# TorchIO-project/torchio

Hardware: NVIDIA H100
Metric: augmented voxels/sec on 256^3 fp32 Compose pipeline (higher is better)
Workload: dtype f32

## Files before the change

### torchio_b200/csrc/build.py

```python

from __future__ import annotations

import os
import subprocess
import sys
from concurrent.futures import ThreadPoolExecutor
from pathlib import Path

HERE = Path(__file__).resolve().parent
ROOT = HERE.parent.parent
SOURCES = ["error.cu", "resample.cu", "resample_tile.cu", "resample_fast.cu", "intensity.cu", "fused_intensity.cu",
           "mt19937_jump.cpp", "mt19937.cu", "patches.cu", "stats.cu", "labels.cu"]
HEADERS = [HERE / "common.cuh", HERE / "intensity_common.cuh", HERE / "resample_common.cuh", HERE / "resample_tile.cuh", HERE / "tma.cuh",
           ROOT / "include" / "tio_b200.h",
           Path(__file__).resolve()]
OBJ = HERE / "_obj"
OUT = HERE / "libtio_b200.so"

ARCH = ["-gencode", "arch=compute_90a,code=sm_90a"]
NVCC_FLAGS = [
    *ARCH,
    "-O3", "-std=c++17", "-lineinfo",
    "-Xcompiler", "-fPIC",
    "-Xptxas", "-v",
]


def needs_build() -> bool:
    if not OUT.exists():
        return True
    newest = max(p.stat().st_mtime for p in [*(HERE / s for s in SOURCES), *HEADERS])
    return OUT.stat().st_mtime < newest


def _compile(source: str) -> tuple[str, int, str]:
    src = HERE / source
    obj = OBJ / (Path(source).stem + ".o")
    newest = max(p.stat().st_mtime for p in [src, *HEADERS])
    if obj.exists() and obj.stat().st_mtime >= newest:
        return source, 0, ""
    proc = subprocess.run(["nvcc", *NVCC_FLAGS, "-c", str(src), "-o", str(obj)],
                          capture_output=True, text=True)
    return source, proc.returncode, proc.stdout + proc.stderr


def build(force: bool = False, verbose: bool = False) -> Path:
    if not force and not needs_build():
        return OUT
    OBJ.mkdir(exist_ok=True)
    if force:
        for stale in OBJ.glob("*.o"):
            stale.unlink()
    with ThreadPoolExecutor(max_workers=min(len(SOURCES), os.cpu_count() or 1)) as pool:
        results = list(pool.map(_compile, SOURCES))
    log = "".join(f"==== {name}\n{text}" for name, _, text in results)
    failed = [name for name, code, _ in results if code != 0]
    if verbose or failed:
        sys.stderr.write(log)
    if failed:
        raise RuntimeError(f"nvcc failed for {failed}")
    objects = [str(OBJ / (Path(s).stem + ".o")) for s in SOURCES]
    proc = subprocess.run(["nvcc", *ARCH, "-shared", "-o", str(OUT),
                           *objects], capture_output=True, text=True)
    if proc.returncode != 0:
        sys.stderr.write(proc.stdout + proc.stderr)
        raise RuntimeError(f"nvcc link failed with exit code {proc.returncode}")
    previous = (HERE / "ptxas.log").read_text() if (HERE / "ptxas.log").exists() and not force else ""
    (HERE / "ptxas.log").write_text(log if all(t for _, _, t in results) else previous + log)
    return OUT


if __name__ == "__main__":
    path = build(force="--force" in sys.argv, verbose="--verbose" in sys.argv)
    print(path)
```

### torchio_b200/csrc/mt19937.cu

```cuda
#include "common.cuh"

namespace tio {

constexpr int MT_N = 624, MT_M = 397, MT_DEG = 19937;
constexpr int MT_SEQ = MT_DEG + MT_N;
constexpr int MT_OFFS = (MT_SEQ + 7) / 4 * 4;

__device__ __forceinline__ uint32_t mt_twist(uint32_t a, uint32_t b, uint32_t c) {
  const uint32_t y = (a & 0x80000000u) | (b & 0x7fffffffu);
  return c ^ (y >> 1) ^ ((y & 1u) ? 0x9908b0dfu : 0u);
}

__device__ __forceinline__ uint32_t mt_temper(uint32_t y) {
  y ^= y >> 11;
  y ^= (y << 7) & 0x9d2c5680u;
  y ^= (y << 15) & 0xefc60000u;
  y ^= y >> 18;
  return y;
}

__global__ void mt_seed_kernel(uint32_t seed, uint32_t* __restrict__ states) {
  if (threadIdx.x == 0) {
    uint32_t v = seed;
    states[0] = v;
    for (int j = 1; j < MT_N; ++j) {
      v = 1812433253u * (v ^ (v >> 30)) + (uint32_t)j;
      states[j] = v;
    }
  }
}

struct MtJob { int src, dst, slot; };

__global__ void __launch_bounds__(640)
mt_jump_kernel(uint32_t* __restrict__ states, const uint16_t* __restrict__ polys, int stride,
               int first, int S2, int fine) {
  extern __shared__ __align__(16) uint32_t seq[];
  uint32_t* offs = seq + MT_OFFS;
  MtJob job;
  if (fine) {
    const int q = first + (int)blockIdx.x, r = q % S2;
    if (r == 0) return;
    job = MtJob{q - r, q, r - 1};
  } else {
    const int m = first + (int)blockIdx.x;
    job = MtJob{0, m * S2, (S2 - 1) + (m - 1)};
  }
  const int tid = threadIdx.x;
  const uint32_t* src = states + (size_t)job.src * MT_N;
  for (int t = tid; t < MT_N; t += blockDim.x) seq[t] = src[t];
  __syncthreads();
  for (int base = 0; base + MT_N < MT_SEQ; base += MT_N - MT_M) {
    const int k = base + tid;
    if (tid < MT_N - MT_M && k + MT_N < MT_SEQ)
      seq[k + MT_N] = mt_twist(seq[k], seq[k + 1], seq[k + MT_M]);
    __syncthreads();
  }
  const uint16_t* p = polys + (size_t)job.slot * stride;
  const uint32_t count = p[0] | ((uint32_t)p[1] << 16);
  const char* mine = reinterpret_cast<const char*>(seq + (tid < MT_N ? tid : 0));
  uint32_t acc = 0;
  for (uint32_t c0 = 0; c0 < count; c0 += 2048) {
    const uint32_t chunk = min(2048u, count - c0);
    for (uint32_t t = tid; t < chunk; t += blockDim.x) offs[t] = (uint32_t)p[2 + c0 + t] << 2;
    __syncthreads();
    if (tid < MT_N) {
      const uint4* o4 = reinterpret_cast<const uint4*>(offs);
      const uint32_t quads = chunk >> 2;
#pragma unroll 4
      for (uint32_t t = 0; t < quads; ++t) {
        const uint4 o = o4[t];
        acc ^= *reinterpret_cast<const uint32_t*>(mine + o.x) ^ *reinterpret_cast<const uint32_t*>(mine + o.y);
        acc ^= *reinterpret_cast<const uint32_t*>(mine + o.z) ^ *reinterpret_cast<const uint32_t*>(mine + o.w);
      }
      for (uint32_t t = quads << 2; t < chunk; ++t) acc ^= *reinterpret_cast<const uint32_t*>(mine + offs[t]);
    }
    __syncthreads();
  }
  if (tid < MT_N) states[(size_t)job.dst * MT_N + tid] = acc;
}

__device__ __forceinline__ void sincos_0_2pi(float theta, float& sn, float& cs) {
  const float t = __fmaf_rn(theta, 0.6366197723675814f, 12582912.0f);
  const int j = __float_as_int(t);
  const float jf = __fsub_rn(t, 12582912.0f);
  float r = __fmaf_rn(jf, -1.5707962512969971f, theta);
  r = __fmaf_rn(jf, -7.549789415861596e-08f, r);
  const float r2 = __fmul_rn(r, r);
  float ps = __fmaf_rn(r2, -1.9515295891e-4f, 8.3321608736e-3f);
  ps = __fmaf_rn(ps, r2, -1.6666654611e-1f);
  const float s = __fmaf_rn(__fmul_rn(ps, r2), r, r);
  float pc = __fmaf_rn(r2, 2.443315711809948e-5f, -1.388731625493765e-3f);
  pc = __fmaf_rn(pc, r2, 4.166664568298827e-2f);
  const float c = __fmaf_rn(__fmul_rn(pc, r2), r2, __fmaf_rn(r2, -0.5f, 1.0f));
  const bool swap = j & 1;
  const float a = swap ? c : s, b = swap ? s : c;
  sn = (j & 2) ? -a : a;
  cs = ((j + 1) & 2) ? -b : b;
}

__global__ void __launch_bounds__(320)
mt_normal_kernel(const uint32_t* __restrict__ states, int q_first, unsigned long long L,
                 unsigned long long offset, unsigned long long n, float* __restrict__ z) {
  __shared__ uint32_t s[2 * MT_N];
  const int tid = threadIdx.x;
  const int q = q_first + blockIdx.x;
  const unsigned long long seg_begin = (unsigned long long)q * L;
  const unsigned long long lo = max(seg_begin, offset);
  const unsigned long long hi = min(seg_begin + L, offset + n);
  if (lo >= hi) return;
  const uint32_t* w = states + (size_t)q * MT_N;
  for (int t = tid; t < MT_N; t += blockDim.x) s[t] = w[t];
  __syncthreads();
  constexpr int W = MT_N - MT_M;
  const int blk = tid >> 3, j = tid & 7;
  const int pair = 16 * blk + j;
  const int lo_rel = (int)(lo - seg_begin), hi_rel = (int)(hi - seg_begin);
  const long long seg_to_z = (long long)seg_begin - (long long)offset;
  int flip = 0;
  for (int base = 0; base < hi_rel; base += MT_N, flip ^= 1) {
    const uint32_t* cur = s + flip * MT_N;
    uint32_t* nxt = s + (flip ^ 1) * MT_N;
    if (tid < W) nxt[tid] = mt_twist(cur[tid], cur[tid + 1], cur[tid + MT_M]);
    __syncthreads();
    if (tid < W) nxt[W + tid] = mt_twist(cur[W + tid], cur[W + tid + 1], nxt[tid]);
    __syncthreads();
    if (tid < MT_N - 2 * W) {
      const int k = 2 * W + tid;
      const uint32_t b = (k + 1 < MT_N) ? cur[k + 1] : nxt[0];
      nxt[k] = mt_twist(cur[k], b, nxt[k - W]);
    }
    __syncthreads();
    if (tid < 312 && base + MT_N > lo_rel) {
      const int t0 = base + pair;
      const bool whole = (base >= lo_rel) && (base + MT_N <= hi_rel);
      if (whole || (t0 >= lo_rel && t0 < hi_rel)) {
        const float u1 = (float)(mt_temper(nxt[pair]) & 0xffffffu) * (1.0f / 16777216.0f);
        const float u2 = (float)(mt_temper(nxt[pair + 8]) & 0xffffffu) * (1.0f / 16777216.0f);
        float radius;
        asm("sqrt.approx.ftz.f32 %0, %1;" : "=f"(radius) : "f"(-2.0f * logf(1.0f - u1)));
        const float theta = (float)(6.283185307179586 * (double)u2);
        float sn, cs;
        sincos_0_2pi(theta, sn, cs);
        float* zp = z + (seg_to_z + t0);
        zp[0] = radius * cs;
        zp[8] = radius * sn;
      }
    }
  }
}

}

using namespace tio;

extern "C" size_t tio_randn_mt19937_workspace_bytes(uint64_t offset, uint64_t n) {
  const uint64_t L = 1ull << 20;
  const uint64_t q_hi = (offset + n + L - 1) / L;
  return (size_t)(q_hi + 64) * MT_N * 4;
}

extern "C" int tio_randn_mt19937(uint64_t seed, uint64_t offset, uint64_t n, float* z,
                                 const void* table, void* workspace, size_t workspace_bytes,
                                 void* stream) {
  TIO_CHECK_ARG(z && table && workspace, "tio_randn_mt19937: null pointer");
  TIO_CHECK_ARG(n >= 16 && (n % 16) == 0 && (offset % 16) == 0,
                "tio_randn_mt19937: n and offset must be multiples of 16 (n >= 16)");
  const uint64_t L = 1ull << 20;
  const int S2 = 32, S1 = 64, stride = 10496;
  const uint64_t q_lo = offset / L, q_hi = (offset + n + L - 1) / L;
  TIO_CHECK_ARG(q_hi <= (uint64_t)S1 * S2, "tio_randn_mt19937: stream position beyond %d segments", S1 * S2);
  TIO_CHECK_ARG(workspace_bytes >= tio_randn_mt19937_workspace_bytes(offset, n),
                "tio_randn_mt19937: workspace too small");
  cudaStream_t st = (cudaStream_t)stream;
  uint32_t* states = (uint32_t*)workspace;
  const uint16_t* polys = (const uint16_t*)((const char*)table + 32);
  mt_seed_kernel<<<1, 32, 0, st>>>((uint32_t)seed, states);
  const size_t jump_smem = (size_t)(MT_OFFS + 2048) * 4;
  cudaFuncSetAttribute(mt_jump_kernel, cudaFuncAttributeMaxDynamicSharedMemorySize, (int)jump_smem);
  const int m_lo = (int)(q_lo / S2), m_hi = (int)((q_hi - 1) / S2);
  const int m_first = m_lo > 1 ? m_lo : 1;
  if (m_hi >= m_first)
    mt_jump_kernel<<<m_hi - m_first + 1, 640, jump_smem, st>>>(states, polys, stride, m_first, S2, 0);
  mt_jump_kernel<<<(unsigned)(q_hi - q_lo), 640, jump_smem, st>>>(states, polys, stride, (int)q_lo, S2, 1);
  mt_normal_kernel<<<(unsigned)(q_hi - q_lo), 320, 0, st>>>(states, (int)q_lo, L, offset, n, z);
  TIO_CHECK_LAUNCH();
  return 0;
}
```

### torchio_b200/csrc/mt19937_jump.cpp

```cpp
#include <stdint.h>
#include <string.h>

#include <vector>

#include "../../include/tio_b200.h"

namespace {

constexpr int kDeg = 19937;
constexpr int kWords = (2 * kDeg + 63) / 64 + 1;

struct Bits {
  std::vector<uint64_t> w;
  explicit Bits(int words = kWords) : w(words, 0) {}
  bool get(int i) const { return (w[i >> 6] >> (i & 63)) & 1u; }
  void flip(int i) { w[i >> 6] ^= (uint64_t)1 << (i & 63); }
  void set(int i) { w[i >> 6] |= (uint64_t)1 << (i & 63); }
};

static void xor_shifted(Bits& a, const Bits& b, int s, int nw) {
  const int ws = s >> 6, bs = s & 63;
  const int limit = (int)a.w.size();
  if (bs == 0) {
    for (int i = 0; i < nw && i + ws < limit; ++i) a.w[i + ws] ^= b.w[i];
  } else {
    for (int i = 0; i < nw; ++i) {
      const uint64_t v = b.w[i];
      if (!v) continue;
      if (i + ws < limit) a.w[i + ws] ^= v << bs;
      if (i + ws + 1 < limit) a.w[i + ws + 1] ^= v >> (64 - bs);
    }
  }
}

struct Mt {
  uint32_t s[624];
  int idx;
  void seed(uint32_t v) {
    s[0] = v;
    for (int j = 1; j < 624; ++j) s[j] = 1812433253u * (s[j - 1] ^ (s[j - 1] >> 30)) + (uint32_t)j;
    idx = 624;
  }
  uint32_t raw() {
    if (idx >= 624) {
      for (int k = 0; k < 624; ++k) {
        uint32_t y = (s[k] & 0x80000000u) | (s[(k + 1) % 624] & 0x7fffffffu);
        s[k] = s[(k + 397) % 624] ^ (y >> 1) ^ ((y & 1u) ? 0x9908b0dfu : 0u);
      }
      idx = 0;
    }
    return s[idx++];
  }
};

struct Field {
  Bits phi;
  std::vector<int> phi_terms;

  void reduce(Bits& a) const {
    for (int d = 2 * kDeg; d >= kDeg; --d) {
      if (!a.get(d)) continue;
      const int s = d - kDeg;
      a.flip(d);
      for (int e : phi_terms) a.flip(e + s);
    }
  }
  Bits mul(const Bits& a, const Bits& b) const {
    Bits r;
    const int nw = (kDeg + 63) / 64;
    for (int i = 0; i < kDeg; ++i)
      if (a.get(i)) xor_shifted(r, b, i, nw);
    reduce(r);
    return r;
  }
};

static bool build_field(Field& f) {
  Mt g;
  g.seed(19650218u);
  std::vector<uint8_t> seq(2 * kDeg + 64);
  for (auto& v : seq) v = (uint8_t)(g.raw() & 1u);
  const int n = (int)seq.size();
  const int W = (kDeg + 64) / 64 + 1;
  std::vector<uint64_t> c(W, 0), b(W, 0), t(W, 0), rev(W, 0);
  c[0] = 1;
  b[0] = 1;
  int L = 0, m = 1;
  for (int i = 0; i < n; ++i) {
    for (int k = W - 1; k > 0; --k) rev[k] = (rev[k] << 1) | (rev[k - 1] >> 63);
    rev[0] = (rev[0] << 1) | seq[i];
    uint64_t acc = 0;
    for (int k = 0; k < W; ++k) acc ^= c[k] & rev[k];
    const int d = __builtin_popcountll(acc) & 1;
    if (d) {
      t = c;
      const int ws = m >> 6, bs = m & 63;
      for (int k = 0; k + ws < W; ++k) {
        c[k + ws] ^= b[k] << bs;
        if (bs && k + ws + 1 < W) c[k + ws + 1] ^= b[k] >> (64 - bs);
      }
      if (2 * L <= i) {
        L = i + 1 - L;
        b = t;
        m = 1;
      } else {
        ++m;
      }
    } else {
      ++m;
    }
  }
  if (L != kDeg) return false;
  f.phi = Bits();
  f.phi_terms.clear();
  for (int j = 0; j <= kDeg; ++j)
    if ((c[j >> 6] >> (j & 63)) & 1u) {
      f.phi.set(kDeg - j);
      if (kDeg - j < kDeg) f.phi_terms.push_back(kDeg - j);
    }
  return f.phi.get(kDeg);
}

}

static constexpr uint32_t kMagic = 0x4d544a31u;
static constexpr int kLog2L = 20, kS2 = 32, kS1 = 64;
static constexpr int kStride = 10496;

extern "C" size_t tio_mt19937_table_bytes(void) {
  return 32 + (size_t)((kS2 - 1) + (kS1 - 1)) * kStride * sizeof(uint16_t);
}

extern "C" int tio_mt19937_build_table(void* blob, size_t bytes) {
  if (!blob || bytes < tio_mt19937_table_bytes()) return 1;
  Field f;
  if (!build_field(f)) return 2;
  uint32_t* header = (uint32_t*)blob;
  header[0] = kMagic; header[1] = kLog2L; header[2] = kS2; header[3] = kS1;
  header[4] = (kS2 - 1) + (kS1 - 1); header[5] = kStride; header[6] = header[7] = 0;
  uint16_t* out = (uint16_t*)((char*)blob + 32);
  auto emit = [&](const Bits& p, int slot) -> bool {
    uint16_t* dst = out + (size_t)slot * kStride;
    uint32_t count = 0;
    for (int i = 0; i < kDeg; ++i)
      if (p.get(i)) {
        if (2 + count >= (uint32_t)kStride) return false;
        dst[2 + count++] = (uint16_t)i;
      }
    dst[0] = (uint16_t)(count & 0xffffu);
    dst[1] = (uint16_t)(count >> 16);
    return true;
  };
  Bits h1;
  h1.set(1);
  for (int i = 0; i < kLog2L; ++i) h1 = f.mul(h1, h1);
  Bits cur = h1;
  for (int r = 1; r < kS2; ++r) {
    if (!emit(cur, r - 1)) return 3;
    cur = f.mul(cur, h1);
  }
  const Bits b1 = cur;
  cur = b1;
  for (int m = 1; m < kS1; ++m) {
    if (!emit(cur, (kS2 - 1) + (m - 1))) return 3;
    if (m + 1 < kS1) cur = f.mul(cur, b1);
  }
  return 0;
}

extern "C" int tio_mt19937_apply_poly_host(const void* blob, int slot, const uint32_t* in,
                                           uint32_t* out) {
  const uint32_t* header = (const uint32_t*)blob;
  if (header[0] != kMagic || slot < 0 || slot >= (int)header[4]) return 1;
  const uint16_t* p = (const uint16_t*)((const char*)blob + 32) + (size_t)slot * header[5];
  const uint32_t count = p[0] | ((uint32_t)p[1] << 16);
  std::vector<uint32_t> seq(kDeg + 624 + 8);
  memcpy(seq.data(), in, 624 * 4);
  for (int k = 0; k + 624 < (int)seq.size(); ++k) {
    uint32_t y = (seq[k] & 0x80000000u) | (seq[k + 1] & 0x7fffffffu);
    seq[k + 624] = seq[k + 397] ^ (y >> 1) ^ ((y & 1u) ? 0x9908b0dfu : 0u);
  }
  for (int j = 0; j < 624; ++j) out[j] = 0;
  for (uint32_t t = 0; t < count; ++t) {
    const uint32_t* s = seq.data() + p[2 + t];
    for (int j = 0; j < 624; ++j) out[j] ^= s[j];
  }
  return 0;
}
```

### torchio_b200/ops.py

```python

from __future__ import annotations

import os
import threading

import numpy as np
import torch
from torch import Tensor

from . import _native

DTYPE_CODES = {
    torch.float32: 0, torch.uint8: 1, torch.int8: 2,
    torch.int16: 3, torch.int32: 4, torch.int64: 5,
}
NEAREST, LINEAR, LABEL_PV = 0, 1, 2
FLAG_PASSTHROUGH, FLAG_ELASTIC = 1, 2

_counter = threading.local()


def launches() -> int:
    return getattr(_counter, "n", 0)


def _count(n: int) -> None:
    _counter.n = getattr(_counter, "n", 0) + n


def _stream(t: Tensor) -> int:
    return torch.cuda.current_stream(t.device).cuda_stream


def _ptr(t: Tensor | None):
    return None if t is None else t.data_ptr()


def _require_cuda(t: Tensor, name: str) -> None:
    if not t.is_cuda:
        raise RuntimeError(
            f"torchio_b200.ops.{name}: expected a CUDA tensor (got {t.device});"
            " the kernels have no CPU fallback"
        )
    if t.requires_grad:
        raise NotImplementedError(
            f"torchio_b200.ops.{name}: kernels are forward-only; detach() the input"
        )


class _StagingRing:

    SLOTS = 64
    SLOT_BYTES = 1 << 20

    def __init__(self) -> None:
        self.buffers = [torch.empty(self.SLOT_BYTES, dtype=torch.uint8, pin_memory=True)
                        for _ in range(self.SLOTS)]
        self.events: list = [None] * self.SLOTS
        self.index = 0
        self.lock = threading.Lock()

    def take(self):
        with self.lock:
            i = self.index
            self.index = (i + 1) % self.SLOTS
            pending, self.events[i] = self.events[i], None
        if pending is not None:
            pending.synchronize()
        return i, self.buffers[i]

    def release(self, i: int, device: torch.device) -> None:
        ev = torch.cuda.Event()
        ev.record(torch.cuda.current_stream(device))
        with self.lock:
            self.events[i] = ev


_ring: _StagingRing | None = None
_init_lock = threading.Lock()


def upload(device: torch.device, *arrays):
    global _ring
    specs, offset = [], 0
    for a in arrays:
        if a is None:
            specs.append(None)
            continue
        t = torch.as_tensor(a)
        t = t.contiguous()
        nbytes = t.numel() * t.element_size()
        specs.append((t, offset, nbytes))
        offset += (nbytes + 15) // 16 * 16
    if offset == 0:
        return [None] * len(arrays)
    slot = None
    if torch.cuda.is_available() and offset <= _StagingRing.SLOT_BYTES:
        if _ring is None:
            with _init_lock:
                if _ring is None:
                    _ring = _StagingRing()
        slot, stage = _ring.take()
        stage = stage[:offset]
    else:
        stage = torch.empty(offset, dtype=torch.uint8, pin_memory=torch.cuda.is_available())
    stage_np = stage.numpy()
    for s in specs:
        if s is None:
            continue
        t, off, nbytes = s
        stage_np[off:off + nbytes] = t.reshape(-1).numpy().view(np.uint8)
    if slot is not None:
        dev = torch.empty(offset, dtype=torch.uint8, device=device)
        _native.call("tio_upload", stage.data_ptr(), dev.data_ptr(), offset,
                     torch.cuda.current_stream(dev.device).cuda_stream)
        _count(1)
        _ring.release(slot, torch.device(device))
    else:
        dev = stage.to(device, non_blocking=True)
    out = []
    for s in specs:
        if s is None:
            out.append(None)
            continue
        t, off, nbytes = s
        out.append(dev[off:off + nbytes].view(t.dtype).reshape(t.shape))
    return out


EXACT_COORDS = 0x100
_exact_default = os.environ.get("TIO_B200_EXACT_COORDS", "0") not in ("", "0")


def set_exact_coords(enabled: bool) -> bool:
    global _exact_default
    previous, _exact_default = _exact_default, bool(enabled)
    return previous


def exact_coords_default() -> bool:
    return _exact_default


def resample(
    src: Tensor, mat: Tensor, cp: Tensor | None, flags: Tensor | None,
    spacing_in, spacing_out, *, affine_first: bool, mode: int,
    fill: Tensor | None, out_shape=None, box_hint: int = 0, exact_coords: bool | None = None,
) -> Tensor:
    _require_cuda(src, "resample")
    if src.dtype not in DTYPE_CODES:
        raise TypeError(f"resample: unsupported dtype {src.dtype}")
    src = src.contiguous()
    b, c, i, j, k = src.shape
    oi, oj, ok = (i, j, k) if out_shape is None else out_shape
    dst = torch.empty((b, c, oi, oj, ok), dtype=src.dtype, device=src.device)
    ni = nj = nk = 0
    if cp is not None:
        ni, nj, nk = cp.shape[1:4]
    sp_in = np.asarray(spacing_in, dtype=np.float32)
    sp_out = np.asarray(spacing_out, dtype=np.float32)
    workspace, ws_bytes = None, 0
    tiled = (src.dtype == torch.float32 and mode == LINEAR) or (
        mode in (NEAREST, LABEL_PV) and src.dtype in (torch.uint8, torch.int16, torch.int32))
    if box_hint >= 0 and tiled:
        ws_bytes = _native.lib().tio_resample_workspace_bytes(b, oi, oj, ok)
        workspace = torch.empty(ws_bytes, dtype=torch.uint8, device=src.device)
    with torch.cuda.device(src.device):
        _native.call(
            "tio_resample", _ptr(src), _ptr(dst), DTYPE_CODES[src.dtype],
            b, c, i, j, k, oi, oj, ok, _ptr(mat), _ptr(cp), _ptr(flags), ni, nj, nk,
            sp_in.ctypes.data, sp_out.ctypes.data, int(bool(affine_first)),
            int(mode) | (EXACT_COORDS if (_exact_default if exact_coords is None else exact_coords) else 0),
            _ptr(fill), int(box_hint), _ptr(workspace), ws_bytes, _stream(src),
        )
    _count(2 if workspace is not None else 1)
    return dst


def _label_table(labels: Tensor, dtype: torch.dtype) -> Tensor:
    return labels.to(torch.float32 if dtype == torch.float32 else torch.int64).contiguous()


def onehot(src: Tensor, labels: Tensor) -> Tensor:
    _require_cuda(src, "onehot")
    if src.dtype not in DTYPE_CODES:
        raise TypeError(f"onehot: unsupported dtype {src.dtype}")
    src = src.contiguous()
    b, n = src.shape[0], int(labels.numel())
    vox = src[0].numel()
    table = _label_table(labels, src.dtype)
    dst = torch.empty((b, n, *src.shape[2:]), dtype=torch.float32, device=src.device)
    with torch.cuda.device(src.device):
        _native.call("tio_onehot", _ptr(src), DTYPE_CODES[src.dtype], b, vox, _ptr(table), n, _ptr(dst),
                     _stream(src))
    _count(1)
    return dst


def label_argmax(sampled: Tensor, labels: Tensor, pad_label: float, dtype: torch.dtype) -> Tensor:
    _require_cuda(sampled, "label_argmax")
    if dtype not in DTYPE_CODES:
        raise TypeError(f"label_argmax: unsupported dtype {dtype}")
    sampled = sampled.contiguous()
    b, n = sampled.shape[:2]
    vox = sampled[0, 0].numel()
    table = _label_table(labels, dtype)
    dst = torch.empty((b, 1, *sampled.shape[2:]), dtype=dtype, device=sampled.device)
    with torch.cuda.device(sampled.device):
        _native.call("tio_label_argmax", _ptr(sampled), b, n, vox, _ptr(table), float(pad_label), _ptr(dst),
                     DTYPE_CODES[dtype], _stream(sampled))
    _count(1)
    return dst


def min_sample0(src: Tensor) -> Tensor:
    _require_cuda(src, "min_sample0")
    src = src.contiguous()
    c = src.shape[1]
    n = src[0, 0].numel()
    fill = torch.empty(c, dtype=torch.float32, device=src.device)
    with torch.cuda.device(src.device):
        _native.call("tio_min_sample0", _ptr(src), c, n, _ptr(fill), _stream(src))
    _count(2)
    return fill


def crop_patches(volume: Tensor, corners, size, out: Tensor | None = None) -> Tensor:
    _require_cuda(volume, "crop_patches")
    if volume.ndim != 4:
        raise ValueError(f"crop_patches expects a (C, I, J, K) volume, got {tuple(volume.shape)}")
    volume = volume.contiguous()
    corners = np.ascontiguousarray(np.asarray(corners, dtype=np.int32).reshape(-1, 3))
    n = corners.shape[0]
    c, i, j, k = (int(v) for v in volume.shape)
    pi, pj, pk = (int(v) for v in size)
    if n == 0:
        return volume.new_empty((0, c, pi, pj, pk))
    if corners.min() < 0 or np.any(corners + np.asarray([pi, pj, pk]) > np.asarray([i, j, k])):
        raise ValueError("crop_patches: a patch extends beyond the volume")
    (corners_d,) = upload(volume.device, corners)
    if out is None:
        dst = torch.empty((n, c, pi, pj, pk), dtype=volume.dtype, device=volume.device)
    else:
        dst = out
        if (tuple(dst.shape) != (n, c, pi, pj, pk) or dst.dtype != volume.dtype or dst.device != volume.device
                or not dst.is_contiguous()):
            raise ValueError("crop_patches: `out` must be a contiguous (n, C, *size) block of the volume's dtype/device")
    with torch.cuda.device(volume.device):
        _native.call(
            "tio_crop_patches", _ptr(volume), _ptr(dst), volume.element_size(), c, i, j, k, n,
            _ptr(corners_d), pi, pj, pk, _stream(volume),
        )
    _count(1)
    return dst


PAD_MODES = {"constant": 0, "replicate": 1, "reflect": 2, "circular": 3}


def remap(src: Tensor, out_shape, offsets, *, mode: str = "constant", fill=0, flip: Tensor | None = None,
          out: Tensor | None = None) -> Tensor:
    _require_cuda(src, "remap")
    if src.ndim != 5:
        raise ValueError(f"remap expects (B, C, I, J, K), got {tuple(src.shape)}")
    src = src.contiguous()
    b, c, i, j, k = (int(v) for v in src.shape)
    oi, oj, ok = (int(v) for v in out_shape)
    if out is None:
        dst = torch.empty((b, c, oi, oj, ok), dtype=src.dtype, device=src.device)
    else:
        dst = out
        if (tuple(dst.shape) != (b, c, oi, oj, ok) or dst.dtype != src.dtype or dst.device != src.device
                or not dst.is_contiguous()):
            raise ValueError("remap: `out` must be a contiguous (B, C, *out_shape) block of the source's dtype/device")
    fill_host = torch.tensor([fill]).to(src.dtype)
    with torch.cuda.device(src.device):
        _native.call(
            "tio_remap", _ptr(src), _ptr(dst), src.element_size(), b, c, i, j, k, oi, oj, ok,
            int(offsets[0]), int(offsets[1]), int(offsets[2]), PAD_MODES[mode],
            fill_host.data_ptr(), _ptr(flip), _stream(src),
        )
    _count(1)
    return dst


def bias_field(src: Tensor, coarse: Tensor, identity: Tensor | None, *, divide=False,
               out: Tensor | None = None) -> Tensor:
    _require_cuda(src, "bias_field")
    src = src.contiguous()
    b, c, i, j, k = src.shape
    dst = torch.empty_like(src) if out is None else out
    si, sj, sk = coarse.shape[2:]
    with torch.cuda.device(src.device):
        _native.call(
            "tio_bias_field", _ptr(src), _ptr(dst), b, c, i, j, k, _ptr(coarse), si, sj, sk,
            _ptr(identity), int(bool(divide)), _stream(src),
        )
    _count(1)
    return dst


def blur(src: Tensor, taps: Tensor, radius: Tensor, big_r: int, axes_mask: int,
         identity: Tensor | None) -> Tensor:
    _require_cuda(src, "blur")
    src = src.contiguous()
    b, c, i, j, k = src.shape
    dst = torch.empty_like(src)
    scratch = torch.empty_like(src) if (axes_mask & 6) else None
    with torch.cuda.device(src.device):
        _native.call(
            "tio_blur", _ptr(src), _ptr(dst), _ptr(scratch), b, c, i, j, k, _ptr(taps),
            _ptr(radius), int(big_r), int(axes_mask), _ptr(identity), _stream(src),
        )
    _count(_fused_launches(axes_mask, False))
    return dst


def _fused_launches(axes_mask: int, has_bias: bool) -> int:
    jk = bool(axes_mask & 6)
    march = (not jk) or bool(axes_mask & 1) or has_bias
    return int(jk) + int(march)


def noise(src: Tensor, mean: Tensor, std: Tensor, keep: Tensor | None, z: Tensor,
          z2: Tensor | None = None) -> Tensor:
    _require_cuda(src, "noise")
    src = src.contiguous()
    dst = torch.empty_like(src)
    with torch.cuda.device(src.device):
        _native.call(
            "tio_noise", _ptr(src), _ptr(dst), src.shape[0], src[0].numel(), _ptr(mean),
            _ptr(std), _ptr(keep), _ptr(z), _ptr(z2), _stream(src),
        )
    _count(1)
    return dst


def noise_philox(src: Tensor, mean: Tensor, std: Tensor, keep: Tensor | None, seed: int,
                 rician: bool = False) -> Tensor:
    _require_cuda(src, "noise_philox")
    src = src.contiguous()
    dst = torch.empty_like(src)
    with torch.cuda.device(src.device):
        _native.call(
            "tio_noise_philox", _ptr(src), _ptr(dst), src.shape[0], src[0].numel(),
            _ptr(mean), _ptr(std), _ptr(keep), int(seed), int(bool(rician)), _stream(src),
        )
    _count(1)
    return dst


def gamma(src: Tensor, gam: Tensor) -> Tensor:
    _require_cuda(src, "gamma")
    src = src.contiguous()
    dst = torch.empty_like(src)
    with torch.cuda.device(src.device):
        _native.call(
            "tio_gamma", _ptr(src), _ptr(dst), src.shape[0], src[0].numel(), _ptr(gam),
            _stream(src),
        )
    _count(1)
    return dst


def moments(values: Tensor, mask: Tensor | None = None) -> tuple[float, float, float]:
    _require_cuda(values, "moments")
    values = values.contiguous()
    m8 = None if mask is None else mask.expand_as(values).contiguous().to(torch.uint8)
    out = torch.empty(3, dtype=torch.float64, device=values.device)
    with torch.cuda.device(values.device):
        _native.call("tio_moments", _ptr(values), _ptr(m8), values.numel(), _ptr(out), _stream(values))
    _count(1)
    s, ss, n = out.tolist()
    return s, ss, n


def quantile_neighbours(values: Tensor, qs, mask: Tensor | None = None):
    _require_cuda(values, "quantile_neighbours")
    values = values.contiguous()
    m8 = None if mask is None else mask.expand_as(values).contiguous().to(torch.uint8)
    qs = np.ascontiguousarray(np.asarray(qs, dtype=np.float64).reshape(-1))
    m = int(qs.shape[0])
    dev = values.device
    vals = torch.empty(2 * m, dtype=torch.float32, device=dev)
    out = torch.empty(m + 1, dtype=torch.float64, device=dev)
    ws_bytes = _native.lib().tio_quantiles_workspace_bytes()
    ws = torch.empty(ws_bytes, dtype=torch.uint8, device=dev)
    with torch.cuda.device(dev):
        _native.call("tio_quantiles", _ptr(values), _ptr(m8), values.numel(), qs.ctypes.data, m, _ptr(vals),
                     _ptr(out), out[m:].data_ptr(), _ptr(ws), ws_bytes, _stream(values))
    _count(8)
    host = out.tolist()
    return vals.tolist(), host[:m], int(host[m])


def rescale(src: Tensor, *, lo: float | None = None, hi: float | None = None, sub=None, div=None, mul=None,
            add=None, keep=None) -> Tensor:
    _require_cuda(src, "rescale")
    src = src.contiguous()
    b = src.shape[0]
    flags = (1 if lo is not None else 0)
    tabs = []
    for bit, table in ((2, sub), (4, div), (8, mul), (16, add)):
        if table is None:
            tabs.append(None)
            continue
        flags |= bit
        arr = np.asarray(table, dtype=np.float32).reshape(-1)
        tabs.append(np.ascontiguousarray(np.broadcast_to(arr, (b,)) if arr.size == 1 else arr))
    keep_np = None if keep is None else np.ascontiguousarray(np.asarray(keep, dtype=np.uint8))
    sub_d, div_d, mul_d, add_d, keep_d = upload(src.device, *tabs, keep_np)
    dst = torch.empty_like(src)
    with torch.cuda.device(src.device):
        _native.call("tio_rescale", _ptr(src), _ptr(dst), b, src[0].numel(),
                     float(lo if lo is not None else 0.0), float(hi if hi is not None else 0.0),
                     _ptr(sub_d), _ptr(div_d), _ptr(mul_d), _ptr(add_d), _ptr(keep_d), flags, _stream(src))
    _count(2)
    return dst


def intensity_fused(
    src: Tensor, *, coarse: Tensor | None = None, bias_identity: Tensor | None = None,
    bias_divide: bool = False, taps: Tensor | None = None, radius: Tensor | None = None,
    big_r: int = 0, axes_mask: int = 0, mean: Tensor | None = None, std: Tensor | None = None,
    keep: Tensor | None = None, z: Tensor | None = None, z2: Tensor | None = None,
    philox_seed: int = 0, noise_mode: int = 0, rician: bool = False,
    gamma: Tensor | None = None,
) -> Tensor:
    _require_cuda(src, "intensity_fused")
    src = src.contiguous()
    b, c, i, j, k = src.shape
    dst = torch.empty_like(src)
    jk = taps is not None and (axes_mask & 6)
    scratch = torch.empty_like(src) if jk else None
    si = sj = sk = 0
    if coarse is not None:
        si, sj, sk = coarse.shape[2:]
    with torch.cuda.device(src.device):
        _native.call(
            "tio_intensity_fused", _ptr(src), _ptr(dst), _ptr(scratch), b, c, i, j, k,
            _ptr(coarse), si, sj, sk, _ptr(bias_identity), int(bool(bias_divide)),
            _ptr(taps), _ptr(radius), int(big_r), int(axes_mask),
            _ptr(mean), _ptr(std), _ptr(keep), _ptr(z), _ptr(z2),
            int(philox_seed) & (2**64 - 1), int(noise_mode), int(bool(rician)),
            _ptr(gamma), _stream(src),
        )
    _count(_fused_launches(axes_mask if taps is not None else 0, coarse is not None))
    return dst



_MT_TABLE_FILE = _native.LIB_PATH.parent / "mt19937_jump.bin"
_mt_host_table: Tensor | None = None
_mt_device_tables: dict = {}
_mt_lock = threading.Lock()
MT_MAX_WORDS = 1 << 31


def mt19937_host_table() -> Tensor:
    global _mt_host_table
    with _mt_lock:
        if _mt_host_table is None:
            lib = _native.lib()
            nbytes = lib.tio_mt19937_table_bytes()
            blob = None
            if _MT_TABLE_FILE.exists() and _MT_TABLE_FILE.stat().st_size == nbytes:
                blob = torch.from_numpy(np.fromfile(_MT_TABLE_FILE, dtype=np.uint8))
            if blob is None:
                blob = torch.zeros(nbytes, dtype=torch.uint8)
                _native.call("tio_mt19937_build_table", blob.data_ptr(), nbytes)
                try:
                    blob.numpy().tofile(_MT_TABLE_FILE)
                except OSError:
                    pass
            _mt_host_table = blob
        return _mt_host_table


def _mt_table(device: torch.device) -> Tensor:
    key = (device.type, device.index)
    table = _mt_device_tables.get(key)
    if table is None:
        with _init_lock:
            table = _mt_device_tables.get(key)
            if table is None:
                table = mt19937_host_table().to(device)
                torch.cuda.synchronize(device)
                _mt_device_tables[key] = table
    return table


def randn_mt19937(seed: int, offset: int, n: int, device, out: Tensor | None = None) -> Tensor:
    device = torch.device(device)
    if n < 16 or n % 16 or offset % 16 or offset + n > MT_MAX_WORDS:
        raise ValueError("randn_mt19937: offset and n must be multiples of 16, n >= 16,"
                         " offset + n <= 2**31")
    z = torch.empty(n, dtype=torch.float32, device=device) if out is None else out
    lib = _native.lib()
    ws_bytes = lib.tio_randn_mt19937_workspace_bytes(offset, n)
    workspace = torch.empty(ws_bytes, dtype=torch.uint8, device=device)
    table = _mt_table(device)
    with torch.cuda.device(device):
        _native.call("tio_randn_mt19937", int(seed) & 0xFFFFFFFF, offset, n, _ptr(z), _ptr(table),
                     _ptr(workspace), ws_bytes, torch.cuda.current_stream(device).cuda_stream)
    _count(4)
    return z
```

Measured before the change: 46.64 billion.

## Warp-specialize MT19937 normal generation and split coarse jump across blocks

Restructures the MT19937 normal kernel into producer warps that twist state into a shared-memory ring and consumer warps that temper and apply vectorized Box-Muller. Named barriers let the twist and the transform overlap. The coarse jump polynomial application is split across several blocks per job, with results combined by atomicXor into memset-zeroed states. Segment length doubles (2^21 with 16 fine steps), which halves fine jumps and gives fewer, longer segments. This trades extra shared memory and synchronization complexity against more parallelism, and needs a regenerated jump table whose header is validated in Python.

Result: faster. 50.02 billion (median of 6 runs) (+7.2%).

```diff
diff --git a/torchio_b200/csrc/build.py b/torchio_b200/csrc/build.py
--- a/torchio_b200/csrc/build.py
+++ b/torchio_b200/csrc/build.py
@@ -12,6 +12,7 @@
 SOURCES = ["error.cu", "resample.cu", "resample_tile.cu", "resample_fast.cu", "intensity.cu", "fused_intensity.cu",
            "mt19937_jump.cpp", "mt19937.cu", "patches.cu", "stats.cu", "labels.cu"]
 HEADERS = [HERE / "common.cuh", HERE / "intensity_common.cuh", HERE / "resample_common.cuh", HERE / "resample_tile.cuh", HERE / "tma.cuh",
+           HERE / "mt19937_layout.h",
            ROOT / "include" / "tio_b200.h",
            Path(__file__).resolve()]
 OBJ = HERE / "_obj"
diff --git a/torchio_b200/csrc/mt19937.cu b/torchio_b200/csrc/mt19937.cu
--- a/torchio_b200/csrc/mt19937.cu
+++ b/torchio_b200/csrc/mt19937.cu
@@ -1,4 +1,5 @@
 #include "common.cuh"
+#include "mt19937_layout.h"
 
 namespace tio {
 
@@ -34,16 +35,17 @@
 
 __global__ void __launch_bounds__(640)
 mt_jump_kernel(uint32_t* __restrict__ states, const uint16_t* __restrict__ polys, int stride,
-               int first, int S2, int fine) {
+               int first, int S2, int fine, int parts) {
   extern __shared__ __align__(16) uint32_t seq[];
   uint32_t* offs = seq + MT_OFFS;
+  const int job_idx = (int)blockIdx.x / parts, part = (int)blockIdx.x % parts;
   MtJob job;
   if (fine) {
-    const int q = first + (int)blockIdx.x, r = q % S2;
+    const int q = first + job_idx, r = q % S2;
     if (r == 0) return;
     job = MtJob{q - r, q, r - 1};
   } else {
-    const int m = first + (int)blockIdx.x;
+    const int m = first + job_idx;
     job = MtJob{0, m * S2, (S2 - 1) + (m - 1)};
   }
   const int tid = threadIdx.x;
@@ -58,10 +60,12 @@
   }
   const uint16_t* p = polys + (size_t)job.slot * stride;
   const uint32_t count = p[0] | ((uint32_t)p[1] << 16);
+  const uint32_t t_begin = (uint32_t)((uint64_t)count * part / parts);
+  const uint32_t t_end = (uint32_t)((uint64_t)count * (part + 1) / parts);
   const char* mine = reinterpret_cast<const char*>(seq + (tid < MT_N ? tid : 0));
   uint32_t acc = 0;
-  for (uint32_t c0 = 0; c0 < count; c0 += 2048) {
-    const uint32_t chunk = min(2048u, count - c0);
+  for (uint32_t c0 = t_begin; c0 < t_end; c0 += 2048) {
+    const uint32_t chunk = min(2048u, t_end - c0);
     for (uint32_t t = tid; t < chunk; t += blockDim.x) offs[t] = (uint32_t)p[2 + c0 + t] << 2;
     __syncthreads();
     if (tid < MT_N) {
@@ -77,7 +81,11 @@
     }
     __syncthreads();
   }
-  if (tid < MT_N) states[(size_t)job.dst * MT_N + tid] = acc;
+  if (tid < MT_N) {
+    uint32_t* dst = states + (size_t)job.dst * MT_N + tid;
+    if (parts == 1) *dst = acc;
+    else atomicXor(dst, acc);
+  }
 }
 
 __device__ __forceinline__ void sincos_0_2pi(float theta, float& sn, float& cs) {
@@ -99,52 +107,108 @@
   cs = ((j + 1) & 2) ? -b : b;
 }
 
-__global__ void __launch_bounds__(320)
+__device__ __forceinline__ void mt_box_muller(uint32_t a, uint32_t b, float& zc, float& zs) {
+  const float u1 = (float)(mt_temper(a) & 0xffffffu) * (1.0f / 16777216.0f);
+  const float u2 = (float)(mt_temper(b) & 0xffffffu) * (1.0f / 16777216.0f);
+  float radius;
+  asm("sqrt.approx.ftz.f32 %0, %1;" : "=f"(radius) : "f"(-2.0f * logf(1.0f - u1)));
+  const float theta = (float)(6.283185307179586 * (double)u2);
+  float sn, cs;
+  sincos_0_2pi(theta, sn, cs);
+  zc = radius * cs;
+  zs = radius * sn;
+}
+
+template <int ID, int COUNT>
+__device__ __forceinline__ void mt_bar_sync() {
+  asm volatile("bar.sync %0, %1;" ::"n"(ID), "n"(COUNT) : "memory");
+}
+template <int ID, int COUNT>
+__device__ __forceinline__ void mt_bar_arrive() {
+  asm volatile("bar.arrive %0, %1;" ::"n"(ID), "n"(COUNT) : "memory");
+}
+
+constexpr int MT_ROUND = 4;
+constexpr int MT_RING = 2 * MT_ROUND;
+constexpr int MT_ITEMS = MT_ROUND * MT_N / 8;
+constexpr int MT_PRODUCERS = 256;
+constexpr int MT_CONSUMERS = (MT_ITEMS + 31) / 32 * 32;
+constexpr int MT_THREADS = MT_PRODUCERS + MT_CONSUMERS;
+constexpr int MT_BAR_PROD = 1, MT_BAR_FULL = 2, MT_BAR_EMPTY = 4;
+
+__global__ void __launch_bounds__(MT_THREADS, 2)
 mt_normal_kernel(const uint32_t* __restrict__ states, int q_first, unsigned long long L,
                  unsigned long long offset, unsigned long long n, float* __restrict__ z) {
-  __shared__ uint32_t s[2 * MT_N];
+  __shared__ __align__(16) uint32_t ring[MT_RING * MT_N];
   const int tid = threadIdx.x;
   const int q = q_first + blockIdx.x;
   const unsigned long long seg_begin = (unsigned long long)q * L;
   const unsigned long long lo = max(seg_begin, offset);
   const unsigned long long hi = min(seg_begin + L, offset + n);
   if (lo >= hi) return;
-  const uint32_t* w = states + (size_t)q * MT_N;
-  for (int t = tid; t < MT_N; t += blockDim.x) s[t] = w[t];
-  __syncthreads();
-  constexpr int W = MT_N - MT_M;
-  const int blk = tid >> 3, j = tid & 7;
-  const int pair = 16 * blk + j;
   const int lo_rel = (int)(lo - seg_begin), hi_rel = (int)(hi - seg_begin);
-  const long long seg_to_z = (long long)seg_begin - (long long)offset;
-  int flip = 0;
-  for (int base = 0; base < hi_rel; base += MT_N, flip ^= 1) {
-    const uint32_t* cur = s + flip * MT_N;
-    uint32_t* nxt = s + (flip ^ 1) * MT_N;
-    if (tid < W) nxt[tid] = mt_twist(cur[tid], cur[tid + 1], cur[tid + MT_M]);
-    __syncthreads();
-    if (tid < W) nxt[W + tid] = mt_twist(cur[W + tid], cur[W + tid + 1], nxt[tid]);
-    __syncthreads();
-    if (tid < MT_N - 2 * W) {
-      const int k = 2 * W + tid;
-      const uint32_t b = (k + 1 < MT_N) ? cur[k + 1] : nxt[0];
-      nxt[k] = mt_twist(cur[k], b, nxt[k - W]);
-    }
-    __syncthreads();
-    if (tid < 312 && base + MT_N > lo_rel) {
-      const int t0 = base + pair;
-      const bool whole = (base >= lo_rel) && (base + MT_N <= hi_rel);
-      if (whole || (t0 >= lo_rel && t0 < hi_rel)) {
-        const float u1 = (float)(mt_temper(nxt[pair]) & 0xffffffu) * (1.0f / 16777216.0f);
-        const float u2 = (float)(mt_temper(nxt[pair + 8]) & 0xffffffu) * (1.0f / 16777216.0f);
-        float radius;
-        asm("sqrt.approx.ftz.f32 %0, %1;" : "=f"(radius) : "f"(-2.0f * logf(1.0f - u1)));
-        const float theta = (float)(6.283185307179586 * (double)u2);
-        float sn, cs;
-        sincos_0_2pi(theta, sn, cs);
-        float* zp = z + (seg_to_z + t0);
-        zp[0] = radius * cs;
-        zp[8] = radius * sn;
+  const int rounds = ((hi_rel + MT_N - 1) / MT_N + MT_ROUND - 1) / MT_ROUND;
+  if (tid < MT_PRODUCERS) {
+    constexpr int W = MT_N - MT_M;
+    const uint32_t* w = states + (size_t)q * MT_N;
+    uint32_t* start = ring + (MT_RING - 1) * MT_N;
+    for (int t = tid; t < MT_N; t += MT_PRODUCERS) start[t] = w[t];
+    mt_bar_sync<MT_BAR_PROD, MT_PRODUCERS>();
+    for (int r = 0; r < rounds; ++r) {
+      if (r >= 2) {
+        if (r & 1) mt_bar_sync<MT_BAR_EMPTY + 1, MT_THREADS>();
+        else mt_bar_sync<MT_BAR_EMPTY, MT_THREADS>();
+      }
+      for (int i = 0; i < MT_ROUND; ++i) {
+        const int b = r * MT_ROUND + i;
+        const uint32_t* cur = ring + ((b + MT_RING - 1) % MT_RING) * MT_N;
+        uint32_t* nxt = ring + (b % MT_RING) * MT_N;
+        if (tid < W) nxt[tid] = mt_twist(cur[tid], cur[tid + 1], cur[tid + MT_M]);
+        mt_bar_sync<MT_BAR_PROD, MT_PRODUCERS>();
+        if (tid < W) nxt[W + tid] = mt_twist(cur[W + tid], cur[W + tid + 1], nxt[tid]);
+        mt_bar_sync<MT_BAR_PROD, MT_PRODUCERS>();
+        if (tid < MT_N - 2 * W) {
+          const int k = 2 * W + tid;
+          const uint32_t c = (k + 1 < MT_N) ? cur[k + 1] : nxt[0];
+          nxt[k] = mt_twist(cur[k], c, nxt[k - W]);
+        }
+        mt_bar_sync<MT_BAR_PROD, MT_PRODUCERS>();
+      }
+      if (r & 1) mt_bar_arrive<MT_BAR_FULL + 1, MT_THREADS>();
+      else mt_bar_arrive<MT_BAR_FULL, MT_THREADS>();
+    }
+  } else {
+    const int c = tid - MT_PRODUCERS;
+    const int blk = c / (MT_N / 8), item = c % (MT_N / 8);
+    const int word = 16 * (item >> 1) + 4 * (item & 1);
+    const long long seg_to_z = (long long)seg_begin - (long long)offset;
+    const bool vec = ((reinterpret_cast<uintptr_t>(z) & 15) == 0);
+    for (int r = 0; r < rounds; ++r) {
+      if (r & 1) mt_bar_sync<MT_BAR_FULL + 1, MT_THREADS>();
+      else mt_bar_sync<MT_BAR_FULL, MT_THREADS>();
+      const int b = r * MT_ROUND + blk;
+      const int group = b * MT_N + (word & ~15);
+      if (c < MT_ITEMS && group >= lo_rel && group < hi_rel) {
+        const uint32_t* x = ring + (b % MT_RING) * MT_N + word;
+        const uint4 a = *reinterpret_cast<const uint4*>(x);
+        const uint4 s = *reinterpret_cast<const uint4*>(x + 8);
+        float4 zc, zs;
+        mt_box_muller(a.x, s.x, zc.x, zs.x);
+        mt_box_muller(a.y, s.y, zc.y, zs.y);
+        mt_box_muller(a.z, s.z, zc.z, zs.z);
+        mt_box_muller(a.w, s.w, zc.w, zs.w);
+        float* zp = z + (seg_to_z + b * MT_N + word);
+        if (vec) {
+          *reinterpret_cast<float4*>(zp) = zc;
+          *reinterpret_cast<float4*>(zp + 8) = zs;
+        } else {
+          zp[0] = zc.x; zp[1] = zc.y; zp[2] = zc.z; zp[3] = zc.w;
+          zp[8] = zs.x; zp[9] = zs.y; zp[10] = zs.z; zp[11] = zs.w;
+        }
+      }
+      if (r + 2 < rounds) {
+        if (r & 1) mt_bar_arrive<MT_BAR_EMPTY + 1, MT_THREADS>();
+        else mt_bar_arrive<MT_BAR_EMPTY, MT_THREADS>();
       }
     }
   }
@@ -154,10 +218,11 @@
 
 using namespace tio;
 
+constexpr uint64_t MT_L = 1ull << tio_mt::kLog2L;
+
 extern "C" size_t tio_randn_mt19937_workspace_bytes(uint64_t offset, uint64_t n) {
-  const uint64_t L = 1ull << 20;
-  const uint64_t q_hi = (offset + n + L - 1) / L;
-  return (size_t)(q_hi + 64) * MT_N * 4;
+  const uint64_t q_hi = (offset + n + MT_L - 1) / MT_L;
+  return (size_t)(q_hi + tio_mt::kS1) * MT_N * 4;
 }
 
 extern "C" int tio_randn_mt19937(uint64_t seed, uint64_t offset, uint64_t n, float* z,
@@ -166,24 +231,28 @@
   TIO_CHECK_ARG(z && table && workspace, "tio_randn_mt19937: null pointer");
   TIO_CHECK_ARG(n >= 16 && (n % 16) == 0 && (offset % 16) == 0,
                 "tio_randn_mt19937: n and offset must be multiples of 16 (n >= 16)");
-  const uint64_t L = 1ull << 20;
-  const int S2 = 32, S1 = 64, stride = 10496;
-  const uint64_t q_lo = offset / L, q_hi = (offset + n + L - 1) / L;
+  const int S2 = tio_mt::kS2, S1 = tio_mt::kS1, stride = tio_mt::kStride;
+  const uint64_t q_lo = offset / MT_L, q_hi = (offset + n + MT_L - 1) / MT_L;
   TIO_CHECK_ARG(q_hi <= (uint64_t)S1 * S2, "tio_randn_mt19937: stream position beyond %d segments", S1 * S2);
   TIO_CHECK_ARG(workspace_bytes >= tio_randn_mt19937_workspace_bytes(offset, n),
                 "tio_randn_mt19937: workspace too small");
   cudaStream_t st = (cudaStream_t)stream;
   uint32_t* states = (uint32_t*)workspace;
-  const uint16_t* polys = (const uint16_t*)((const char*)table + 32);
+  const uint16_t* polys = (const uint16_t*)((const char*)table + tio_mt::kHeaderBytes);
   mt_seed_kernel<<<1, 32, 0, st>>>((uint32_t)seed, states);
   const size_t jump_smem = (size_t)(MT_OFFS + 2048) * 4;
   cudaFuncSetAttribute(mt_jump_kernel, cudaFuncAttributeMaxDynamicSharedMemorySize, (int)jump_smem);
   const int m_lo = (int)(q_lo / S2), m_hi = (int)((q_hi - 1) / S2);
   const int m_first = m_lo > 1 ? m_lo : 1;
-  if (m_hi >= m_first)
-    mt_jump_kernel<<<m_hi - m_first + 1, 640, jump_smem, st>>>(states, polys, stride, m_first, S2, 0);
-  mt_jump_kernel<<<(unsigned)(q_hi - q_lo), 640, jump_smem, st>>>(states, polys, stride, (int)q_lo, S2, 1);
-  mt_normal_kernel<<<(unsigned)(q_hi - q_lo), 320, 0, st>>>(states, (int)q_lo, L, offset, n, z);
+  if (m_hi >= m_first) {
+    constexpr int kCoarseParts = 8;
+    const size_t pitch = (size_t)S2 * MT_N * 4;
+    cudaMemset2DAsync(states + (size_t)m_first * S2 * MT_N, pitch, 0, MT_N * 4, m_hi - m_first + 1, st);
+    mt_jump_kernel<<<(m_hi - m_first + 1) * kCoarseParts, 640, jump_smem, st>>>(states, polys, stride, m_first,
+                                                                             S2, 0, kCoarseParts);
+  }
+  mt_jump_kernel<<<(unsigned)(q_hi - q_lo), 640, jump_smem, st>>>(states, polys, stride, (int)q_lo, S2, 1, 1);
+  mt_normal_kernel<<<(unsigned)(q_hi - q_lo), MT_THREADS, 0, st>>>(states, (int)q_lo, MT_L, offset, n, z);
   TIO_CHECK_LAUNCH();
   return 0;
 }
diff --git a/torchio_b200/csrc/mt19937_jump.cpp b/torchio_b200/csrc/mt19937_jump.cpp
--- a/torchio_b200/csrc/mt19937_jump.cpp
+++ b/torchio_b200/csrc/mt19937_jump.cpp
@@ -4,6 +4,7 @@
 #include <vector>
 
 #include "../../include/tio_b200.h"
+#include "mt19937_layout.h"
 
 namespace {
 
@@ -123,12 +124,14 @@
 
 }
 
-static constexpr uint32_t kMagic = 0x4d544a31u;
-static constexpr int kLog2L = 20, kS2 = 32, kS1 = 64;
-static constexpr int kStride = 10496;
+using tio_mt::kLog2L;
+using tio_mt::kMagic;
+using tio_mt::kS1;
+using tio_mt::kS2;
+using tio_mt::kStride;
 
 extern "C" size_t tio_mt19937_table_bytes(void) {
-  return 32 + (size_t)((kS2 - 1) + (kS1 - 1)) * kStride * sizeof(uint16_t);
+  return tio_mt::kHeaderBytes + (size_t)tio_mt::kPolys * kStride * sizeof(uint16_t);
 }
 
 extern "C" int tio_mt19937_build_table(void* blob, size_t bytes) {
@@ -137,8 +140,8 @@
   if (!build_field(f)) return 2;
   uint32_t* header = (uint32_t*)blob;
   header[0] = kMagic; header[1] = kLog2L; header[2] = kS2; header[3] = kS1;
-  header[4] = (kS2 - 1) + (kS1 - 1); header[5] = kStride; header[6] = header[7] = 0;
-  uint16_t* out = (uint16_t*)((char*)blob + 32);
+  header[4] = tio_mt::kPolys; header[5] = kStride; header[6] = header[7] = 0;
+  uint16_t* out = (uint16_t*)((char*)blob + tio_mt::kHeaderBytes);
   auto emit = [&](const Bits& p, int slot) -> bool {
     uint16_t* dst = out + (size_t)slot * kStride;
     uint32_t count = 0;
@@ -172,7 +175,7 @@
                                            uint32_t* out) {
   const uint32_t* header = (const uint32_t*)blob;
   if (header[0] != kMagic || slot < 0 || slot >= (int)header[4]) return 1;
-  const uint16_t* p = (const uint16_t*)((const char*)blob + 32) + (size_t)slot * header[5];
+  const uint16_t* p = (const uint16_t*)((const char*)blob + tio_mt::kHeaderBytes) + (size_t)slot * header[5];
   const uint32_t count = p[0] | ((uint32_t)p[1] << 16);
   std::vector<uint32_t> seq(kDeg + 624 + 8);
   memcpy(seq.data(), in, 624 * 4);
diff --git a/torchio_b200/csrc/mt19937_layout.h b/torchio_b200/csrc/mt19937_layout.h
--- /dev/null
+++ b/torchio_b200/csrc/mt19937_layout.h
@@ -0,0 +1,13 @@
+#pragma once
+
+#include <stdint.h>
+
+namespace tio_mt {
+
+constexpr uint32_t kMagic = 0x4d544a31u;
+constexpr int kLog2L = 21, kS2 = 16, kS1 = 64;
+constexpr int kStride = 10496;
+constexpr int kPolys = (kS2 - 1) + (kS1 - 1);
+constexpr int kHeaderBytes = 32;
+
+}
diff --git a/torchio_b200/ops.py b/torchio_b200/ops.py
--- a/torchio_b200/ops.py
+++ b/torchio_b200/ops.py
@@ -455,6 +455,7 @@
 _mt_device_tables: dict = {}
 _mt_lock = threading.Lock()
 MT_MAX_WORDS = 1 << 31
+MT_TABLE_HEADER = (0x4D544A31, 21, 16, 64, 78, 10496)
 
 
 def mt19937_host_table() -> Tensor:
@@ -465,7 +466,9 @@
             nbytes = lib.tio_mt19937_table_bytes()
             blob = None
             if _MT_TABLE_FILE.exists() and _MT_TABLE_FILE.stat().st_size == nbytes:
-                blob = torch.from_numpy(np.fromfile(_MT_TABLE_FILE, dtype=np.uint8))
+                cached = np.fromfile(_MT_TABLE_FILE, dtype=np.uint8)
+                if tuple(int(v) for v in cached[:24].view(np.uint32)) == MT_TABLE_HEADER:
+                    blob = torch.from_numpy(cached)
             if blob is None:
                 blob = torch.zeros(nbytes, dtype=torch.uint8)
                 _native.call("tio_mt19937_build_table", blob.data_ptr(), nbytes)
```
